# lizhiqi49/threestudio-3dgs

Hardware: AMD Instinct MI355X
Metric: rendered views/sec fwd+bwd @1M Gaussians, 1024², SH=3; 1/2/4/8 GPU (higher is better)
Workload: dtype fp32

## Files before the change

### threestudio-3dgs_amd/csrc/gsr_api.hip

```cpp
#include <stdio.h>
#include <string.h>

#include <cmath>
#include <mutex>
#include <vector>

#include "../../include/gsr.h"
#include "gsr_kernels.h"

using namespace gsr;

static thread_local char g_err[512] = "";

static int fail(int code, const char* fmt, const char* what) {
  snprintf(g_err, sizeof(g_err), fmt, what);
  return code;
}

#define GSR_HIP_CHECK(expr)                                                        \
  do {                                                                             \
    hipError_t e_ = (expr);                                                        \
    if (e_ != hipSuccess) return fail(GSR_EHIP, "HIP error: %s", hipGetErrorString(e_)); \
  } while (0)

// ... 1008 lines not shown
      state->image == nullptr || gr.work == nullptr || dL_dcolor == nullptr || gr.dL_dmeans2D == nullptr ||
      gr.dL_dcolors == nullptr || gr.dL_dopacity == nullptr || gr.dL_dmeans3D == nullptr ||
      state->radii == nullptr || sc.means3D == nullptr)
    return fail(GSR_EINVAL, "%s", "null pointer argument");
  if (sc.shs != nullptr && gr.dL_dsh == nullptr) return fail(GSR_EINVAL, "%s", "dL_dsh required with SHs");
  if (sc.cov3D_precomp == nullptr && (sc.scales == nullptr || sc.rotations == nullptr || gr.dL_dscales == nullptr ||
                                      gr.dL_drotations == nullptr))
    return fail(GSR_EINVAL, "%s", "scales/rotations and their gradients required");
  SetCams cams;
  if (set_cams(sc, cams) != GSR_OK) return GSR_EINVAL;
  SegInfo inst;
  long long total = 0;
  if (inst_segments(V, K, inst, &total) != GSR_OK) return GSR_EINVAL;
  hipStream_t s = (hipStream_t)stream;
  GeomState g = GeomState::carve(state->geom, V, P, nullptr);
  const TilePack tp = set_tile_pack(P, width, height);
  BinningState b = BinningState::carve(state->binning, V, total, inst.blk[V], !tp.packed, nullptr);
  ImageState img = ImageState::carve(state->image, V, width, height, nullptr, true);
  const int gx = div_up(width, GSR_TILE_X), gy = div_up(height, GSR_TILE_Y);
  const size_t HW = (size_t)width * height;
  const int tres = tile_sort_result(width, height);
  const uint32_t* sorted = tp.packed ? b.key[tres] : b.val[tres];
  GaussBackwardArgs a = shared_args(sc, gr);
  if (gr.accumulate != 0 && sc.cov3D_precomp == nullptr && dL_dcov3D == nullptr)
    return fail(GSR_EINVAL, "%s", "accumulate needs dL_dcov3D: it carries the running dL/dcov3D between calls");
  void* work = gr.work;
  if (gr.work_bytes < carry_bytes(P)) return fail(GSR_EINVAL, "%s", "backward work buffer too small");
  const size_t avail = (gr.work_bytes - carry_bytes(P)) & ~(size_t)255;
  float* carry = dL_dcov3D ? dL_dcov3D : (float*)((char*)work + avail);
  bool first = gr.accumulate == 0;
  for (int g0 = 0; g0 < V;) {
    int g1 = g0;
    long long rows = 0;
    while (g1 < V && (g1 == g0 || BackwardState::bytes_for(rows + K[g1], g1 + 1 - g0, P, two) <= avail))
      rows += K[g1++];
    if (BackwardState::bytes_for(rows, g1 - g0, P, two) > avail)
      return fail(GSR_EINVAL, "%s", "backward work buffer smaller than one view's gradient rows");
    BackwardState bw = BackwardState::carve(work, rows, P, two);
    RenderSet rs;
    rs.cbg = comp_bg ? comp_bg + (size_t)g0 * HW * 3 : nullptr;
    rs.comp = nullptr;
    rs.ccolor = color ? color + (size_t)g0 * 3 * HW : nullptr;
    rs.dcbg = dL_dbg ? dL_dbg + (size_t)g0 * HW * 3 : nullptr;
    rs.col2 = two ? gr.colors2 : colors_override;
    rs.col2_rec = g.drange + 130;
    rs.out_col2 = nullptr;
    rs.dpix2 = two ? gr.dL_dcolor2 + (size_t)g0 * 3 * HW : nullptr;
    rs.order = img.order;
    rs.ckpt = !two && colors_override == nullptr && split_fits(V, (size_t)gx * gy) ? img.ckpt : nullptr;
    rs.split_mode = img.split_mode;
    rs.split_items = img.split_items;
    rs.split_cap = img.split_cap;
    rs.split_extra = split_extra(V, (size_t)gx * gy);
    rs.qkeys = tp.qmask ? b.key[tres] : nullptr;
    rs.qbytes = reinterpret_cast<uint8_t*>(b.key[tres ^ 1]);
    rs.V = g1 - g0;
    rs.ochunk = order_chunk(rs.V, gx, gy, false);
    rs.v0 = g0;
    rs.P = P;
    rs.W = width;
    rs.H = height;
    rs.gx = gx;
    rs.gy = gy;
    rs.gmask = tp.gmask;
    ViewGradArgs va;
    va.V = g1 - g0;
    va.v0 = g0;
    va.W = width;
    va.H = height;
    va.gx = gx;
    va.tiles = gx * gy;
    va.cut_in_lds = 0;
    va.items = 0;
    va.g = g;
    va.img = img;
    va.reach = bw.reach;
    va.grow = bw.grow;
    va.dmeans2D = gr.dL_dmeans2D;
    va.vrec = bw.vrec;
    AccumArgs ab;
    ab.V = g1 - g0;
    ab.v0 = g0;
    ab.accumulate = first ? 0 : 1;
    ab.pad_ = 0;
    ab.reach = bw.reach;
    ab.vrec = bw.vrec;
    ab.dcov_carry = carry;
    ab.dcolors2 = two ? gr.dL_dcolors2 : nullptr;
    for (int v = g0; v < g1; ++v) {
      if (bgs[v] == nullptr) return fail(GSR_EINVAL, "%s", "null background");
      rs.inst_start[v - g0] = inst.start[v];
      rs.row_start[v - g0] = inst.start[v] - inst.start[g0];
      rs.bg[v - g0] = bgs[v];
      va.row_start[v - g0] = rs.row_start[v - g0];
      va.cam[v - g0] = cams.c[v];
      ab.campos[v - g0] = cams.c[v].campos;
    }
    {
      PhaseScope ps(GSR_PHASE_RENDER_BWD, s);
      GSR_HIP_CHECK(hipMemsetAsync(bw.reach, 0, sizeof(unsigned long long) * (size_t)P, s));
      launch_render_backward(rs, g, sorted, img, dL_dcolor + (size_t)g0 * 3 * HW,
                             dL_ddepth ? dL_ddepth + (size_t)g0 * HW : nullptr,
                             dL_dalpha ? dL_dalpha + (size_t)g0 * HW : nullptr, bw, s);
    }
    {
      PhaseScope ps(GSR_PHASE_GAUSS_BWD, s);
      const bool last = g1 == V;
      if (last && gr.n_chunks > 0) {
        const int cs = grad_chunk_size(P, gr.n_chunks);
        for (int c = 0; c < gr.n_chunks; ++c) {
          GaussBackwardArgs ac = a;
          ac.g0 = c * cs < P ? c * cs : P;
          ac.g1 = (c + 1) * cs < P ? (c + 1) * cs : P;
          launch_gauss_backward(ac, va, ab, s);
          if (gr.chunk_events[c] != nullptr) GSR_HIP_CHECK(hipEventRecord((hipEvent_t)gr.chunk_events[c], s));
        }
      } else {
        launch_gauss_backward(a, va, ab, s);
      }
    }
    first = false;
    g0 = g1;
  }
  return last_launch();
}

int gsr_grad_chunk_range(int P, int n_chunks, int chunk, int* g0, int* g1) {
  if (P < 0 || n_chunks < 1 || n_chunks > GSR_GRAD_CHUNKS_MAX || chunk < 0 || chunk >= n_chunks || g0 == nullptr ||
      g1 == nullptr)
    return fail(GSR_EINVAL, "%s", "bad gradient chunk query");
  const int cs = grad_chunk_size(P, n_chunks);
  *g0 = chunk * cs < P ? chunk * cs : P;
  *g1 = (chunk + 1) * cs < P ? (chunk + 1) * cs : P;
  return GSR_OK;
}


size_t gsr_geom_bytes(int P) { return gsr_set_geom_bytes(1, P); }
size_t gsr_binning_bytes(int K, int width, int height) {
  SegInfo seg;
  long long total = 0;
  if (K < 0 || inst_segments(1, &K, seg, &total) != GSR_OK) return 0;
  size_t b = 0;
  BinningState::carve(nullptr, 1, total, seg.blk[1], true, &b);
  return b;
}
size_t gsr_image_bytes(int width, int height) { return gsr_set_image_bytes(1, 0, nullptr, width, height, 0); }
size_t gsr_backward_bytes(int P, int K) { return gsr_set_backward_bytes(1, P, &K, 0); }

int gsr_forward_preprocess(int P, int degree, int M, const float* means3D, const float* scales,
                           float scale_modifier, const float* rotations, const float* opacities,
                           const float* shs, const float* colors_precomp, const float* cov3D_precomp,
                           const float* viewmatrix, const float* projmatrix, const float* campos,
                           int width, int height, float tanfovx, float tanfovy, int prefiltered,
                           int* radii, void* geom, void* stream) {
  const gsr_set_scene sc{1, P, degree, M, width, height, prefiltered, scale_modifier, means3D, scales, rotations,
                         opacities, shs, colors_precomp, cov3D_precomp, &viewmatrix, &projmatrix, &campos, nullptr,
                         &tanfovx, &tanfovy};
  const gsr_set_state st{radii, geom, nullptr, nullptr, nullptr};
  return gsr_set_preprocess(&sc, &st, nullptr, stream);
}

int gsr_num_rendered(const void* geom, int P, int* num_rendered, int* num_visible, void* stream) {
  return gsr_set_num_rendered(1, geom, P, num_rendered, num_visible, nullptr, stream);
}

int gsr_forward_render(int P, int K, int width, int height, const float* bg, void* geom,
// ... 81 lines not shown
```

### threestudio-3dgs_amd/csrc/gsr_backward.hip

```cpp
#include <cstdlib>
#include <cstring>

#include "gsr_kernels.h"
#include "gsr_math.h"
#include "gsr_wave.h"

namespace gsr {

struct RowSums {
  float dmx, dmy, dca, dcb, dcc, dop, dcr, dcg, dcbl, ddep;
  float dmx1, dmy1, dr2, dg2, db2;
};

template <bool TWO>
__device__ __forceinline__ RowSums gather_rows(uint32_t idx, const GaussRec& gr, uint32_t i0, int grid_x,
                                               const uint2* cut, const float4* grow) {
  RowSums r = {0.f, 0.f, 0.f, 0.f, 0.f, 0.f, 0.f, 0.f, 0.f, 0.f, 0.f, 0.f, 0.f, 0.f, 0.f};
  constexpr int RW = TWO ? 4 : 3;
  const uint4 gd = gr.d;
  const float4 ga = gr.a, gb = gr.b;
  const uint32_t dkey = __float_as_uint(gb.z);
  const int xmin = gd.x & 0xffff, ymin = gd.x >> 16, xmax = gd.y & 0xffff, ymax = gd.y >> 16;
  const int w = xmax - xmin;
  const SpanPrep sp = span_prep(ga.x, ga.y, ga.z, ga.w, gb.x, gb.y);
// ... 253 lines not shown
#pragma unroll
  for (int it = 0; it < GSR_VG_ITEMS; ++it) {
    const int local = it * 256 + t;
    const int idx = slice + local;
    const bool valid = it < items && idx < a.g1;
    const bool rch = valid && (va.reach[idx] & vbit) != 0ull;
    if (valid && !rch) {
      float* m2 = va.dmeans2D + 3 * ((size_t)vg * a.P + idx);
      m2[0] = 0.f;
      m2[1] = 0.f;
      m2[2] = 0.f;
    }
    const unsigned long long bal = __ballot(rch);
    if (rch) list[cnt + mask_rank(bal)] = (uint16_t)local;
    cnt += __popcll(bal);
  }
  asm volatile("s_waitcnt lgkmcnt(0)" ::: "memory");
  GaussRec nrec;
  uint32_t ngo = 0u;
  int nidx = 0;
  if (lane < cnt) {
    nidx = slice + list[lane];
    const size_t o0 = (size_t)vg * a.P + nidx;
    nrec = va.g.rec[o0], ngo = va.g.goff[o0];
  }
#pragma unroll 1
  for (int i = lane; i - lane < cnt; i += 64) {
    if (i >= cnt) break;
    const int idx = nidx;
    const size_t o = (size_t)vg * a.P + idx;
    const GaussRec gr = nrec;
    const uint32_t go = ngo;
    if (i + 64 < cnt) {
      nidx = slice + list[i + 64];
      const size_t on = (size_t)vg * a.P + nidx;
      nrec = va.g.rec[on], ngo = va.g.goff[on];
    }
    float* m2 = va.dmeans2D + 3 * o;
    float4* rec = recv + (size_t)idx * (RS / 4);
    const uint32_t clamp_bits = gr.d.w;
    const RowSums r = gather_rows<TWO>((uint32_t)idx, gr, go, va.gx, cut, grow);
    bool reached = (r.dmx != 0.f) | (r.dmy != 0.f) | (r.dca != 0.f) | (r.dcb != 0.f) | (r.dcc != 0.f) |
                   (r.dop != 0.f) | (r.dcr != 0.f) | (r.dcg != 0.f) | (r.dcbl != 0.f) | (r.ddep != 0.f);
    if (TWO) reached = reached | (r.dr2 != 0.f) | (r.dg2 != 0.f) | (r.db2 != 0.f);
    if (!reached) {
      m2[0] = 0.f;
      m2[1] = 0.f;
      m2[2] = 0.f;
#pragma unroll
      for (int q = 0; q < RS / 4; ++q)
        rec[q] = q == 3 ? make_float4(0.f, __uint_as_float(clamp_bits), 0.f, 0.f) : make_float4(0.f, 0.f, 0.f, 0.f);
      continue;
    }
    m2[0] = TWO ? r.dmx1 : r.dmx;
    m2[1] = TWO ? r.dmy1 : r.dmy;
    m2[2] = 0.f;
    const float3 mean = make_float3(a.means3D[3 * idx], a.means3D[3 * idx + 1], a.means3D[3 * idx + 2]);
    float cov3D[6];
    if (a.cov3D_precomp) {
#pragma unroll
      for (int k = 0; k < 6; ++k) cov3D[k] = a.cov3D_precomp[6 * idx + k];
    } else {
      const float3 scale = make_float3(a.scales[3 * idx], a.scales[3 * idx + 1], a.scales[3 * idx + 2]);
      const float4 rot = make_float4(a.rotations[4 * idx], a.rotations[4 * idx + 1], a.rotations[4 * idx + 2],
                                     a.rotations[4 * idx + 3]);
      cov3d_from_scale_rot(scale, a.scale_modifier, rot, cov3D);
    }
    float dcv[6];
    float3 dm;
    cov2d_backward(mean, cov3D, vgm, r.dca, r.dcb, r.dcc, dcv, dm);
    proj_backward(mean, projm, r.dmx, r.dmy, dm);
    dm.x += viewm[2] * r.ddep;
    dm.y += viewm[6] * r.ddep;
    dm.z += viewm[10] * r.ddep;
    const float f[GSR_REC_STRIDE2] = {dm.x,   dm.y,  dm.z,  dcv[0], dcv[1], dcv[2], dcv[3],
                                      dcv[4], dcv[5], r.dcr, r.dcg,  r.dcbl, r.dop,  __uint_as_float(clamp_bits),
                                      r.dr2,  r.dg2, r.db2, 0.f,   0.f,    0.f};
#pragma unroll
    for (int q = 0; q < RS / 4; ++q) rec[q] = make_float4(f[4 * q], f[4 * q + 1], f[4 * q + 2], f[4 * q + 3]);
  }
}

__attribute__((amdgpu_waves_per_eu(3, 8)))
__global__ __launch_bounds__(256) void k_gauss_accum(GaussBackwardArgs a, AccumArgs b) {
  extern __shared__ __attribute__((aligned(16))) float s_sh[];
  const int t = threadIdx.x;
  const int block0 = a.g0 + blockIdx.x * 256;
  const int idx = block0 + t;
  const int nblk = min(256, a.g1 - block0);
  const int F = 3 * a.M;
  const int S = sh_lds_stride(a.M);
  const bool has_sh = a.shs != nullptr && F > 0;
  const bool acc = b.accumulate != 0;
  const float invF = has_sh ? 1.0f / (float)F : 0.0f;
  __shared__ uint8_t s_rl[256];
  __shared__ int s_wcnt[4];
  const unsigned long long reach_word = idx < a.g1 ? b.reach[idx] : 0ull;
  const bool reached = reach_word != 0ull;
  int nr = 0;
  if (has_sh) {
    const unsigned long long bal = __ballot(reached);
    const int w = t >> 6;
    if ((t & 63) == 0) s_wcnt[w] = (int)__popcll(bal);
    __syncthreads();
    int base = 0;
    for (int k = 0; k < 4; ++k) {
      base += k < w ? s_wcnt[k] : 0;
      nr += s_wcnt[k];
    }
    if (reached) s_rl[base + mask_rank(bal)] = (uint8_t)t;
    __syncthreads();
    const int cnt = nr * F;
    for (int e = t; e < cnt; e += 256) {
      const int r = (int)(((float)e + 0.5f) * invF);
      const int tl = s_rl[r];
      const int k = e - r * F;
      s_sh[tl * S + k] = a.shs[(size_t)(block0 + tl) * F + k];
    }
    __syncthreads();
  }
  if (idx < a.g1 && !reached) {
    if (!acc) {
      for (int k = 0; k < 3; ++k) a.dL_dmeans3D[3 * idx + k] = 0.f;
      a.dL_dopacity[idx] = 0.f;
      if (a.dL_dcolors)
        for (int k = 0; k < 3; ++k) a.dL_dcolors[3 * idx + k] = 0.f;
      if (b.dcolors2)
        for (int k = 0; k < 3; ++k) b.dcolors2[3 * idx + k] = 0.f;
      if (b.dcov_carry)
        for (int k = 0; k < 6; ++k) b.dcov_carry[6 * idx + k] = 0.f;
      if (a.dL_dcov3D && a.dL_dcov3D != b.dcov_carry)
        for (int k = 0; k < 6; ++k) a.dL_dcov3D[6 * idx + k] = 0.f;
      if (!a.cov3D_precomp && a.dL_dscales) {
        for (int k = 0; k < 3; ++k) a.dL_dscales[3 * idx + k] = 0.f;
        for (int k = 0; k < 4; ++k) a.dL_drotations[4 * idx + k] = 0.f;
      }
      if (has_sh) {
        float* row = s_sh + t * S;
        for (int k = 0; k < F; ++k) row[k] = 0.f;
      }
    }
  } else if (idx < a.g1) {
    const float3 mean = make_float3(a.means3D[3 * idx], a.means3D[3 * idx + 1], a.means3D[3 * idx + 2]);
    float3 dmean = make_float3(0.f, 0.f, 0.f);
    float dcov[6] = {0.f, 0.f, 0.f, 0.f, 0.f, 0.f};
    float dop = 0.f, dcr = 0.f, dcg = 0.f, dcb = 0.f;
    float dsh[48];
#pragma unroll
    for (int k = 0; k < 48; ++k) dsh[k] = 0.f;
    if (acc) {
      dmean = make_float3(a.dL_dmeans3D[3 * idx], a.dL_dmeans3D[3 * idx + 1], a.dL_dmeans3D[3 * idx + 2]);
      dop = a.dL_dopacity[idx];
      if (a.dL_dcolors) dcr = a.dL_dcolors[3 * idx], dcg = a.dL_dcolors[3 * idx + 1], dcb = a.dL_dcolors[3 * idx + 2];
      if (b.dcov_carry)
#pragma unroll
        for (int k = 0; k < 6; ++k) dcov[k] = b.dcov_carry[6 * idx + k];
      if (has_sh) {
        const float* prev = a.dL_dsh + (size_t)idx * F;
#pragma unroll
        for (int k = 0; k < 48; ++k)
          if (k < F) dsh[k] = prev[k];
      }
    }
    const float* sh_row = has_sh ? s_sh + t * S : nullptr;
    const int RS = b.dcolors2 ? GSR_REC_STRIDE2 : GSR_REC_STRIDE;
    float d2[3] = {0.f, 0.f, 0.f};
    if (b.dcolors2 && acc)
      for (int k = 0; k < 3; ++k) d2[k] = b.dcolors2[3 * idx + k];
    unsigned long long pending = reach_word;
    auto next_view = [&]() -> int {
      if (pending == 0ull) return -1;
      const int v = __builtin_ctzll(pending);
      pending &= pending - 1ull;
      return v;
    };
    auto load = [&](float4 (&f)[4], int vl) {
      const float4* src = reinterpret_cast<const float4*>(b.vrec + ((size_t)vl * a.P + idx) * RS);
#pragma unroll
      for (int q = 0; q < 4; ++q) f[q] = src[q];
    };
    auto process = [&](const float4 (&f4)[4], int vl) {
      const float f[16] = {f4[0].x, f4[0].y, f4[0].z, f4[0].w, f4[1].x, f4[1].y, f4[1].z, f4[1].w,
                           f4[2].x, f4[2].y, f4[2].z, f4[2].w, f4[3].x, f4[3].y, f4[3].z, f4[3].w};
      dmean.x += f[0];
      dmean.y += f[1];
      dmean.z += f[2];
#pragma unroll
      for (int k = 0; k < 6; ++k) dcov[k] += f[3 + k];
      dcr += f[9];
      dcg += f[10];
      dcb += f[11];
      dop += f[12];
      if (b.dcolors2) {
        d2[0] += f[14];
        d2[1] += f[15];
        d2[2] += b.vrec[((size_t)vl * a.P + idx) * RS + 16];
      }
      if (has_sh && ((f[9] != 0.f) | (f[10] != 0.f) | (f[11] != 0.f))) {
        const uint32_t cl = __float_as_uint(f[13]);
        const float3 dRGB = make_float3((cl & 1u) ? 0.f : f[9], (cl & 2u) ? 0.f : f[10], (cl & 4u) ? 0.f : f[11]);
        const float* shv = sh_row;
        typedef __attribute__((address_space(4))) const float* cfptr;
        const float cpos[3] = {((cfptr)b.campos[vl])[0], ((cfptr)b.campos[vl])[1], ((cfptr)b.campos[vl])[2]};
        sh_backward(a.deg, a.M, shv, dsh, dRGB, mean, cpos, dmean);
      }
    };
    float4 fa[4], fb[4];
    int va_ = next_view(), vb_ = next_view();
    if (va_ >= 0) load(fa, va_);
    if (vb_ >= 0) load(fb, vb_);
    for (;;) {
      if (va_ < 0) break;
      process(fa, va_);
      va_ = next_view();
      if (va_ >= 0) load(fa, va_);
      if (vb_ < 0) break;
      process(fb, vb_);
      vb_ = next_view();
      if (vb_ >= 0) load(fb, vb_);
    }
    a.dL_dmeans3D[3 * idx] = dmean.x;
    a.dL_dmeans3D[3 * idx + 1] = dmean.y;
    a.dL_dmeans3D[3 * idx + 2] = dmean.z;
    a.dL_dopacity[idx] = dop;
    if (a.dL_dcolors) {
      a.dL_dcolors[3 * idx] = dcr;
      a.dL_dcolors[3 * idx + 1] = dcg;
      a.dL_dcolors[3 * idx + 2] = dcb;
    }
    if (b.dcolors2)
      for (int k = 0; k < 3; ++k) b.dcolors2[3 * idx + k] = d2[k];
    if (b.dcov_carry)
      for (int k = 0; k < 6; ++k) b.dcov_carry[6 * idx + k] = dcov[k];
    if (a.dL_dcov3D && a.dL_dcov3D != b.dcov_carry)
      for (int k = 0; k < 6; ++k) a.dL_dcov3D[6 * idx + k] = dcov[k];
    if (!a.cov3D_precomp && a.dL_dscales) {
      const float3 scale = make_float3(a.scales[3 * idx], a.scales[3 * idx + 1], a.scales[3 * idx + 2]);
      const float4 rot = make_float4(a.rotations[4 * idx], a.rotations[4 * idx + 1], a.rotations[4 * idx + 2],
                                     a.rotations[4 * idx + 3]);
      float ds[3], dq[4];
      scale_rot_backward(scale, rot, a.scale_modifier, dcov, ds, dq);
      for (int k = 0; k < 3; ++k) a.dL_dscales[3 * idx + k] = ds[k];
      for (int k = 0; k < 4; ++k) a.dL_drotations[4 * idx + k] = dq[k];
    }
    if (has_sh) {
      float* row = s_sh + t * S;
      float4* row4w = reinterpret_cast<float4*>(row);
#pragma unroll
      for (int c = 0; c < 12; ++c)
        if (4 * c < F) row4w[c] = make_float4(dsh[4 * c], dsh[4 * c + 1], dsh[4 * c + 2], dsh[4 * c + 3]);
      for (int k = 48; k < F; ++k) row[k] = 0.f;
    }
  }
  if (has_sh) {
    __syncthreads();
    if (!acc) {
      float* dst = a.dL_dsh + (size_t)block0 * F;
      const int cnt = nblk * F;
      for (int e = t; e < cnt; e += 256) {
        const int te = (int)(((float)e + 0.5f) * invF);
        dst[e] = s_sh[te * S + (e - te * F)];
      }
    } else {
      const int cnt = nr * F;
      for (int e = t; e < cnt; e += 256) {
        const int r = (int)(((float)e + 0.5f) * invF);
        const int tl = s_rl[r];
        const int k = e - r * F;
        a.dL_dsh[(size_t)(block0 + tl) * F + k] = s_sh[tl * S + k];
      }
    }
  }
}

template <bool TWO>
__global__ __launch_bounds__(256) void k_gauss_fused(GaussBackwardArgs a, ViewGradArgs va, AccumArgs b) {
  const int idx = a.g0 + blockIdx.x * 256 + threadIdx.x;
  const bool valid = idx < a.g1;
  const int ix = valid ? idx : a.g0;
  const bool acc = b.accumulate != 0;
  const unsigned long long reach_word = valid ? va.reach[ix] : 0ull;
  float3 dmean = make_float3(0.f, 0.f, 0.f);
  float dcov[6] = {0.f, 0.f, 0.f, 0.f, 0.f, 0.f};
  float dop = 0.f, dcr = 0.f, dcg = 0.f, dcb = 0.f;
  float d2[3] = {0.f, 0.f, 0.f};
  if (valid && acc) {
    dmean = make_float3(a.dL_dmeans3D[3 * idx], a.dL_dmeans3D[3 * idx + 1], a.dL_dmeans3D[3 * idx + 2]);
    dop = a.dL_dopacity[idx];
    if (a.dL_dcolors) dcr = a.dL_dcolors[3 * idx], dcg = a.dL_dcolors[3 * idx + 1], dcb = a.dL_dcolors[3 * idx + 2];
    if (b.dcov_carry)
#pragma unroll
      for (int k = 0; k < 6; ++k) dcov[k] = b.dcov_carry[6 * idx + k];
    if (TWO)
      for (int k = 0; k < 3; ++k) d2[k] = b.dcolors2[3 * idx + k];
  }
  const float3 mean = make_float3(a.means3D[3 * ix], a.means3D[3 * ix + 1], a.means3D[3 * ix + 2]);
  float cov3D[6];
  if (reach_word != 0ull) {
    if (a.cov3D_precomp) {
#pragma unroll
      for (int k = 0; k < 6; ++k) cov3D[k] = a.cov3D_precomp[6 * ix + k];
    } else {
      const float3 scale = make_float3(a.scales[3 * ix], a.scales[3 * ix + 1], a.scales[3 * ix + 2]);
      const float4 rot = make_float4(a.rotations[4 * ix], a.rotations[4 * ix + 1], a.rotations[4 * ix + 2],
                                     a.rotations[4 * ix + 3]);
      cov3d_from_scale_rot(scale, a.scale_modifier, rot, cov3D);
    }
  }
  GaussRec nrec;
  uint32_t ngo = 0u;
  auto fetch = [&](int vl) {
    const size_t o = (size_t)(va.v0 + vl) * a.P + ix;
    nrec = va.g.rec[o];
    ngo = va.g.goff[o];
  };
  const int vfirst = reach_word != 0ull ? (int)__builtin_ctzll(reach_word) : va.V;
  if (vfirst < va.V) fetch(vfirst);
#pragma unroll 1
  for (int vl = 0; vl < va.V; ++vl) {
    const int vg = va.v0 + vl;
    float* m2 = va.dmeans2D + 3 * ((size_t)vg * a.P + ix);
    if (!((reach_word >> vl) & 1ull)) {
      if (valid) m2[0] = 0.f, m2[1] = 0.f, m2[2] = 0.f;
      continue;
    }
    const GaussRec gr = nrec;
    const uint32_t go = ngo;
    const unsigned long long later = reach_word & ~((2ull << vl) - 1ull);
    if (later != 0ull) fetch((int)__builtin_ctzll(later));
    const ViewCam& cam = va.cam[vl];
    typedef __attribute__((address_space(4))) const float* cfptr;
    float viewm[16], projm[16];
#pragma unroll
    for (int i = 0; i < 16; ++i) viewm[i] = ((cfptr)cam.view)[i], projm[i] = ((cfptr)cam.proj)[i];
    ViewGeom vgm;
    vgm.view = viewm;
    vgm.proj = projm;
    vgm.tanx = cam.tanx;
    vgm.tany = cam.tany;
    vgm.fy = va.H / (2.0f * cam.tany);
    vgm.fx = va.W / (2.0f * cam.tanx);
    const float4* grow = va.grow + (size_t)(TWO ? 4 : 3) * va.row_start[vl];
    const uint2* cut = va.img.cut + (size_t)vg * va.tiles;
    const RowSums r = gather_rows<TWO>((uint32_t)ix, gr, go, va.gx, cut, grow);
    bool reached = (r.dmx != 0.f) | (r.dmy != 0.f) | (r.dca != 0.f) | (r.dcb != 0.f) | (r.dcc != 0.f) |
                   (r.dop != 0.f) | (r.dcr != 0.f) | (r.dcg != 0.f) | (r.dcbl != 0.f) | (r.ddep != 0.f);
    if (TWO) reached = reached | (r.dr2 != 0.f) | (r.dg2 != 0.f) | (r.db2 != 0.f);
    if (!reached) {
      if (valid) m2[0] = 0.f, m2[1] = 0.f, m2[2] = 0.f;
      continue;
    }
    if (valid) {
      m2[0] = TWO ? r.dmx1 : r.dmx;
      m2[1] = TWO ? r.dmy1 : r.dmy;
      m2[2] = 0.f;
    }
    float dcv[6];
    float3 dm;
    cov2d_backward(mean, cov3D, vgm, r.dca, r.dcb, r.dcc, dcv, dm);
    proj_backward(mean, projm, r.dmx, r.dmy, dm);
    dm.x += viewm[2] * r.ddep;
    dm.y += viewm[6] * r.ddep;
    dm.z += viewm[10] * r.ddep;
    dmean.x += dm.x;
    dmean.y += dm.y;
    dmean.z += dm.z;
#pragma unroll
    for (int k = 0; k < 6; ++k) dcov[k] += dcv[k];
    dcr += r.dcr;
    dcg += r.dcg;
    dcb += r.dcbl;
    dop += r.dop;
    if (TWO) {
      d2[0] += r.dr2;
      d2[1] += r.dg2;
      d2[2] += r.db2;
    }
  }
  if (!valid) return;
  a.dL_dmeans3D[3 * idx] = dmean.x;
  a.dL_dmeans3D[3 * idx + 1] = dmean.y;
  a.dL_dmeans3D[3 * idx + 2] = dmean.z;
  a.dL_dopacity[idx] = dop;
  if (a.dL_dcolors) {
    a.dL_dcolors[3 * idx] = dcr;
    a.dL_dcolors[3 * idx + 1] = dcg;
    a.dL_dcolors[3 * idx + 2] = dcb;
  }
  if (TWO)
    for (int k = 0; k < 3; ++k) b.dcolors2[3 * idx + k] = d2[k];
  if (b.dcov_carry)
    for (int k = 0; k < 6; ++k) b.dcov_carry[6 * idx + k] = dcov[k];
  if (a.dL_dcov3D && a.dL_dcov3D != b.dcov_carry)
    for (int k = 0; k < 6; ++k) a.dL_dcov3D[6 * idx + k] = dcov[k];
  if (!a.cov3D_precomp && a.dL_dscales) {
    const float3 scale = make_float3(a.scales[3 * idx], a.scales[3 * idx + 1], a.scales[3 * idx + 2]);
    const float4 rot = make_float4(a.rotations[4 * idx], a.rotations[4 * idx + 1], a.rotations[4 * idx + 2],
                                   a.rotations[4 * idx + 3]);
    float ds[3], dq[4];
    scale_rot_backward(scale, rot, a.scale_modifier, dcov, ds, dq);
    for (int k = 0; k < 3; ++k) a.dL_dscales[3 * idx + k] = ds[k];
    for (int k = 0; k < 4; ++k) a.dL_drotations[4 * idx + k] = dq[k];
  }
}

static bool gauss_fused_on(const GaussBackwardArgs& a) {
  if (a.shs != nullptr && a.M > 0) return false;
  const char* e = getenv("GSR_GAUSS_FUSED");
  return !(e != nullptr && strcmp(e, "0") == 0);
}

#define GSR_CUT_LDS_MAX (48 * 1024)

void launch_gauss_backward(const GaussBackwardArgs& a, ViewGradArgs va, const AccumArgs& b, hipStream_t stream) {
  const int n = a.g1 - a.g0;
  if (n <= 0 || va.V <= 0) return;
  if (gauss_fused_on(a)) {
    auto kern = b.dcolors2 ? k_gauss_fused<true> : k_gauss_fused<false>;
    hipLaunchKernelGGL(kern, dim3(div_up(n, 256)), dim3(256), 0, stream, a, va, b);
    return;
  }
  const size_t cut_bytes = sizeof(uint2) * (size_t)va.tiles;
  va.cut_in_lds = cut_bytes <= GSR_CUT_LDS_MAX ? 1 : 0;
  va.items = GSR_VG_ITEMS;
  while (va.items > 2 && (long long)va.V * div_up(n, 256 * va.items) < 1024) va.items >>= 1;
  const dim3 vg_grid(va.V * div_up(n, 256 * va.items));
  auto vg_kern = b.dcolors2 ? (va.cut_in_lds ? k_view_grad<true, true> : k_view_grad<true, false>)
                            : (va.cut_in_lds ? k_view_grad<false, true> : k_view_grad<false, false>);
  hipLaunchKernelGGL(vg_kern, vg_grid, dim3(256), va.cut_in_lds ? cut_bytes : 0, stream, a, va);
  const size_t lds = (a.shs && a.M > 0) ? (size_t)256 * sh_lds_stride(a.M) * sizeof(float) : 0;
  hipLaunchKernelGGL(k_gauss_accum, dim3(div_up(n, 256)), dim3(256), lds, stream, a, b);
}

}
```

### threestudio-3dgs_amd/csrc/gsr_kernels.h

```cpp
#pragma once

#include "gsr_common.h"

namespace gsr {

int seg_sort(uint32_t* keys[2], uint32_t* vals[2], bool vals_identity, SegInfo seg, int bit_lo, int key_bits,
             uint32_t* counts, uint32_t* totals, hipStream_t stream, int max_bits = GSR_RADIX_BITS);
int sort_rank_mode();

struct PreprocessArgs {
  int V, P, deg, M;
  const float *means3D, *scales, *rotations, *opacities, *shs, *colors_precomp, *cov3D_precomp;
  float scale_modifier;
  int W, H;
  int* radii;
  const float* col2;
};
void launch_preprocess(const PreprocessArgs& a, const SetCams& cams, const GeomState& g, hipStream_t stream);

void launch_binning_counts(int V, int P, const GeomState& g, hipStream_t stream);
void launch_emit(int V, int P, int W, const GeomState& g, const SegInfo& inst, const TilePack& tp, uint32_t* keys,
                 uint32_t* vals, hipStream_t stream);
void launch_tile_ranges(SegInfo inst, int n_tiles, const TilePack& tp, const uint32_t* keys, uint2* ranges,
                        hipStream_t stream);
void launch_mark_visible(int P, const float* means3D, const float* view, const float* proj,
                         uint8_t* present, hipStream_t stream);

__device__ __forceinline__ float quad_form(float a, float b, float c, float u, float v) {
  return fmaf(a * u, u, fmaf(2.0f * b * u, v, c * v * v));
}
__device__ __forceinline__ bool quadrant_hit(const float4 r0, const float4 r1, float qx, float qy) {
  const float o = r1.y;
  if (!(o >= GSR_ALPHA_MIN * 0.9999f)) return false;
  const float a = r0.z, b = r0.w, c = r1.x;
  if (!(a > 0.0f && c > 0.0f && a * c - b * b > 0.0f)) return true;
  const float tau = fmaxf(0.0f, __logf(255.0f * o));
  const float thr = 2.0f * (tau * 1.002f + 2e-3f);
  const float u1 = r0.x - qx, u0 = u1 - 7.0f;
  const float v1 = r0.y - qy, v0 = v1 - 7.0f;
  if (u0 <= 0.0f && u1 >= 0.0f && v0 <= 0.0f && v1 >= 0.0f) return true;
  const float ia = 1.0f / a, ic = 1.0f / c;
  const float q0 = quad_form(a, b, c, u0, fminf(fmaxf(-b * u0 * ic, v0), v1));
  const float q1 = quad_form(a, b, c, u1, fminf(fmaxf(-b * u1 * ic, v0), v1));
  const float q2 = quad_form(a, b, c, fminf(fmaxf(-b * v0 * ia, u0), u1), v0);
  const float q3 = quad_form(a, b, c, fminf(fmaxf(-b * v1 * ia, u0), u1), v1);
  const float qmin = fminf(fminf(q0, q1), fminf(q2, q3));
  return qmin * 0.998f <= thr;
}

struct RenderSet {
  int V, v0, P, W, H, gx, gy;
  uint32_t gmask;
  uint32_t inst_start[GSR_SET_MAX];
  uint32_t row_start[GSR_SET_MAX];
  const float* bg[GSR_SET_MAX];
  const float* cbg;
  float* comp;
  const float* ccolor;
  float* dcbg;
  const float* col2;
  float* out_col2;
  const float* dpix2;
  const uint32_t* order;
  int ochunk;
  float* ckpt;
  const uint32_t* split_mode;
  const uint32_t* col2_rec;
  uint32_t* split_items;
  uint32_t* split_cap;
  int split_extra;
  const uint32_t* qkeys;
  uint8_t* qbytes;
};
bool split_on(int V, int P, int width, int height, long long instances);
bool fwd_tile_chosen(long long instances, long long gaussians, int views);
int order_chunk(int V, int gx, int gy, bool forward);
const char* blend_kernel_name(int which);
inline bool split_forward(int V, int P, int width, int height, long long instances, bool two_colors) {
  return !two_colors && split_on(V, P, width, height, instances);
}
void launch_tile_order(int V, int gx, int gy, const uint2* ranges, uint32_t* order, hipStream_t stream);
void launch_render_forward(const RenderSet& rs, const GeomState& g, const uint32_t* sorted_gauss,
                           const ImageState& img, float* out_color, float* out_depth, float* out_alpha,
                           long long instances, hipStream_t stream);
void launch_render_backward(const RenderSet& rs, const GeomState& g, const uint32_t* sorted_gauss,
                            const ImageState& img, const float* dL_dcolor, const float* dL_ddepth,
                            const float* dL_dalpha, const BackwardState& bw, hipStream_t stream);

struct GaussBackwardArgs {
  int P, deg, M;
  int g0, g1;
  const float *means3D, *scales, *rotations, *shs, *cov3D_precomp;
  float scale_modifier;
  float *dL_dcolors, *dL_dopacity, *dL_dmeans3D, *dL_dcov3D, *dL_dsh, *dL_dscales, *dL_drotations;
};
struct ViewGradArgs {
  int V, v0, W, H, gx, tiles, cut_in_lds, items;
  GeomState g;
  ImageState img;
  const unsigned long long* reach;
  const float4* grow;
  float* dmeans2D;
  float* vrec;
  uint32_t row_start[GSR_SET_MAX];
  ViewCam cam[GSR_SET_MAX];
};
struct AccumArgs {
  int V, v0, accumulate, pad_;
  const unsigned long long* reach;
  const float* vrec;
  float* dcov_carry;
  float* dcolors2;
  const float* campos[GSR_SET_MAX];
};
void launch_composite_fwd(int V, size_t HW, const float* color, const float* alpha, const float* bg, int layout,
                          float* out, hipStream_t stream);
void launch_composite_bwd(int V, size_t HW, const float* dout, const float* color, const float* alpha,
                          const float* bg, int layout, float* dcolor, float* dalpha, float* dbg,
                          hipStream_t stream);
void launch_normal_map_fwd(int V, size_t HW, const float* normal, const float* alpha, float* out, hipStream_t stream);
void launch_normal_map_bwd(int V, size_t HW, const float* dout, const float* normal, const float* alpha,
                           float* dnormal, float* dalpha, hipStream_t stream);
struct ShadeArgs {
  int V, v0, H, W, flags, bg_layout;
  const float* color;
  const float* depth;
  const float* alpha;
  const float* rays_o;
  const float* rays_d;
  const float* bg;
  const float* light;
  const float* pred_normal;
  float ka[GSR_SET_MAX][3], kd[GSR_SET_MAX][3];
  int mode[GSR_SET_MAX];
  float* render;
  float* nmap;
  float* unit;
  float* depth_out;
};
struct ShadeGrads {
  const float* d_render;
  const float* d_nmap;
  const float* d_unit;
  const float* d_depth_out;
  float* d_color;
  float* d_depth;
  float* d_alpha;
  float* d_bg;
};
void launch_shade_fwd(const ShadeArgs& A, hipStream_t stream);
void launch_shade_bwd(const ShadeArgs& A, const ShadeGrads& G, hipStream_t stream);
size_t knn_workspace_bytes(int P);
int launch_knn_mean_dist(int P, const float* points, float* out, void* workspace, hipStream_t stream);
int launch_knn_points(int P, int K, const float* points, float* dists, long long* idx, void* workspace,
                      hipStream_t stream);
struct FieldCall {
  int M, K, N, R;
  const float* x;
  const long long *nbr, *row;
  const float *centers, *inv_sr, *strengths, *min_scale;
  float density_factor;
};
size_t field_workspace_bytes(long long M, int K, int N);
int field_gauss_lanes(long long M, int K, int N);
void launch_field_forward(const FieldCall& c, float* density, float* beta_avg, float* op, void* workspace,
                          hipStream_t stream);
int launch_field_backward(const FieldCall& c, const float* g_density, const float* g_beta, const float* g_op, float* dx,
                          float* dcenters, float* dinv_sr, float* dstrengths, float* dmin_scale, void* workspace,
                          hipStream_t stream);
struct NormalCall {
  int M, K, N, R;
  const float* x;
  const long long *own, *nbr;
  int per_sample;
  const float *centers, *normals, *min_scale, *op;
};
size_t normal_workspace_bytes(long long M, int K, int N);
int normal_gauss_lanes(long long M, int K, int N);
void launch_normal_forward(const NormalCall& c, float* loss, float* rec, void* workspace, hipStream_t stream);
int launch_normal_backward(const NormalCall& c, const float* rec, const float* g_loss, float* dnormals,
                           void* workspace, hipStream_t stream);
struct MeshCall {
  int V, F, G;
  const float* verts;
  const int* faces;
  const float *cplx, *log_scales;
};
size_t mesh_workspace_bytes(int F, int V);
void launch_mesh_forward(const MeshCall& c, const float* bary, float thickness, float* xyz, float* scaling,
                         float* rotation, float* normals, hipStream_t stream);
void launch_mesh_backward(const MeshCall& c, const float* bary, const int* corner_order, const int* vert_offsets,
// ... 38 lines not shown
```

Measured before the change: 3988.

## Balance per-Gaussian accumulation work across wavefronts by sorting on reached-view count

The Gaussian gradient accumulation kernel drops from 256-thread blocks to single-wave 64-thread blocks. Four of these waves share each 256-Gaussian chunk, and each wave recomputes a counting sort of the chunk by popcount of the per-Gaussian view-reach mask. Gaussians that touch a similar number of views therefore land in the same wave, which is meant to cut time lanes spend idle behind the longest per-view loop. SH staging in LDS is compacted to reached Gaussians only, and unreached SH gradients are zeroed directly in global memory. The cost is the sort done redundantly in each block, scattered rather than contiguous SH writes, and smaller blocks. A diagnostic script measuring lane imbalance is also added.

```diff
diff --git a/profiles/diag_lane_balance.py b/profiles/diag_lane_balance.py
--- /dev/null
+++ b/profiles/diag_lane_balance.py
@@ -0,0 +1,130 @@
+import ctypes
+import json
+import os
+import sys
+
+ROOT = os.path.dirname(os.path.dirname(os.path.abspath(__file__)))
+sys.path.insert(0, os.path.join(ROOT, "threestudio-3dgs_amd"))
+sys.path.insert(0, ROOT)
+
+import numpy as np
+import torch
+
+import bench
+import gsr_synthetic as gs
+from diff_gaussian_rasterization import _C
+
+
+def popcount64(x: torch.Tensor) -> torch.Tensor:
+    m1, m2, m4 = 0x5555555555555555, 0x3333333333333333, 0x0F0F0F0F0F0F0F0F
+    lo = x & 0xFFFFFFFF
+    hi = (x >> 32) & 0xFFFFFFFF
+    out = 0
+    for h in (lo, hi):
+        h = h - ((h >> 1) & (m1 & 0xFFFFFFFF))
+        h = (h & (m2 & 0xFFFFFFFF)) + ((h >> 2) & (m2 & 0xFFFFFFFF))
+        h = (h + (h >> 4)) & (m4 & 0xFFFFFFFF)
+        out = out + ((h * 0x01010101) >> 24 & 0xFF)
+    return out
+
+
+def pad_to(x: torch.Tensor, m: int) -> torch.Tensor:
+    n = (-x.shape[-1]) % m
+    return torch.nn.functional.pad(x, (0, n)) if n else x
+
+
+def main():
+    lib = _C.load_library()
+    dev = torch.device("cuda", 0)
+    V, R, P = 64, 1024, 1_000_000
+    scene = gs.make_scene(P, sh_degree=3, seed=0)
+    rep = bench.Replica(scene, dev)
+    cams = bench.build_views(V, R, dev)
+    bg0 = torch.zeros(3, device=dev)
+    settings = [bench.settings_for(rep, c, bg0) for c in cams]
+    gen = torch.Generator(device=dev).manual_seed(7)
+    bg_img = torch.rand((V, R, R, 3), generator=gen, device=dev)
+    ups = [torch.randn((V, 3, R, R), generator=gen, device=dev), torch.randn((V, 1, R, R), generator=gen, device=dev),
+           torch.randn((V, 1, R, R), generator=gen, device=dev)]
+
+    hip = ctypes.CDLL("libamdhip64.so")
+    hip.hipMemcpy.argtypes = [ctypes.c_void_p, ctypes.c_void_p, ctypes.c_size_t, ctypes.c_int]
+    inner = lib.gsr_set_backward
+    seen = []
+
+    def set_backward(sc, st, g, stream):
+        rc = inner(sc, st, g, stream)
+        if rc == 0:
+            reach = np.zeros(sc.P, np.int64)
+            assert hip.hipMemcpy(reach.ctypes.data, g.work, 8 * sc.P, 2) == 0
+            rows, vis = geom_state(lib, st.geom, sc.V, sc.P, dev)
+            seen.append((reach, rows, vis, sc.V))
+        return rc
+
+    lib.gsr_set_backward = set_backward
+    c, d, a, _ = bench.render_views(rep, settings, bg_img)
+    torch.autograd.backward((c, d, a), ups)
+    torch.cuda.synchronize()
+    lib.gsr_set_backward = inner
+    assert len(seen) == 1, f"expected one set, saw {len(seen)} backward calls"
+    reach, rows, vis, Vs = seen[0]
+
+    pc = popcount64(torch.from_numpy(reach).to(dev))
+    group_views = (int(np.bitwise_or.reduce(reach)) & (2 ** 64 - 1)).bit_length()
+    hist = torch.bincount(pc, minlength=65).cpu().tolist()
+    waves = pad_to(pc, 64).view(-1, 64)
+    wave_max = int(waves.max(1).values.sum())
+    blocks = pad_to(pc, 256).view(-1, 256)
+    ordered = blocks.sort(1, descending=True).values.reshape(-1, 64)
+    wave_max_ordered = int(ordered.max(1).values.sum())
+    n_waves = waves.shape[0]
+    total = int(pc.sum())
+
+    r = pad_to(torch.where(vis, rows, torch.zeros_like(rows)), 64).view(Vs, -1, 64)
+    row_sum = int(r.sum())
+    row_max64 = int(r.max(2).values.sum()) * 64
+    items = int(vis.sum())
+
+    out = {
+        "workload": f"bench.py default: 1M Gaussians, {R}x{R}, SH3, {V}-view set, fused background composite",
+        "build_id": _C.build_id(lib),
+        "views": Vs,
+        "gauss_accum": {
+            "views_in_last_group": group_views,
+            "popcount_histogram": hist,
+            "mean_popcount": total / P,
+            "reached_fraction": float((pc > 0).float().mean()),
+            "waves": n_waves,
+            "sum_wave_max": wave_max,
+            "sum_wave_max_ordered_256": wave_max_ordered,
+            "sum_wave_mean": total / 64.0,
+            "max_over_ordered": wave_max / max(1, wave_max_ordered),
+            "max_over_mean": wave_max / max(1.0, total / 64.0),
+        },
+        "preprocess": {
+            "visible_nonzero_area": items,
+            "mean_rows": row_sum / max(1, items),
+            "sum_rows": row_sum,
+            "sum_wave_max_x64": row_max64,
+            "max64_over_sum": row_max64 / max(1, row_sum),
+            "mean_wave_max": row_max64 / 64 / (Vs * r.shape[1]),
+            "mean_wave_rounds_of_64": float(((r.sum(2) + 63) // 64).float().mean()),
+        },
+    }
+    path = sys.argv[1] if len(sys.argv) > 1 else os.path.join(ROOT, "profiles", "lane_balance.json")
+    with open(path, "w") as f:
+        json.dump(out, f, indent=1)
+    print(json.dumps(out, indent=1))
+
+
+def geom_state(lib, geom, V, P, dev):
+    rec = torch.zeros((V, P, 16), dtype=torch.float32, device=dev)
+    tiles = torch.zeros((V, P, 2), dtype=torch.int32, device=dev)
+    _C._check(lib.gsr_set_gauss_state(V, geom, P, _C._ptr(rec), _C._ptr(tiles), _C._stream(dev)))
+    d = rec.view(torch.int32)
+    rows = ((d[:, :, 13] >> 16) & 0xFFFF) - ((d[:, :, 12] >> 16) & 0xFFFF)
+    return rows.long(), tiles[:, :, 0] > 0
+
+
+if __name__ == "__main__":
+    main()
diff --git a/threestudio-3dgs_amd/csrc/gsr_api.hip b/threestudio-3dgs_amd/csrc/gsr_api.hip
--- a/threestudio-3dgs_amd/csrc/gsr_api.hip
+++ b/threestudio-3dgs_amd/csrc/gsr_api.hip
@@ -1114,7 +1114,7 @@
     ab.V = g1 - g0;
     ab.v0 = g0;
     ab.accumulate = first ? 0 : 1;
-    ab.pad_ = 0;
+    ab.balance = 0;
     ab.reach = bw.reach;
     ab.vrec = bw.vrec;
     ab.dcov_carry = carry;
diff --git a/threestudio-3dgs_amd/csrc/gsr_backward.hip b/threestudio-3dgs_amd/csrc/gsr_backward.hip
--- a/threestudio-3dgs_amd/csrc/gsr_backward.hip
+++ b/threestudio-3dgs_amd/csrc/gsr_backward.hip
@@ -359,44 +359,83 @@
 }
 
 __attribute__((amdgpu_waves_per_eu(3, 8)))
-__global__ __launch_bounds__(256) void k_gauss_accum(GaussBackwardArgs a, AccumArgs b) {
+__global__ __launch_bounds__(64) void k_gauss_accum(GaussBackwardArgs a, AccumArgs b) {
   extern __shared__ __attribute__((aligned(16))) float s_sh[];
-  const int t = threadIdx.x;
-  const int block0 = a.g0 + blockIdx.x * 256;
-  const int idx = block0 + t;
-  const int nblk = min(256, a.g1 - block0);
+  const int lane = threadIdx.x;
+  const int block0 = a.g0 + (int)(blockIdx.x >> 2) * 256;
+  const int p = (int)(blockIdx.x & 3u);
   const int F = 3 * a.M;
   const int S = sh_lds_stride(a.M);
   const bool has_sh = a.shs != nullptr && F > 0;
   const bool acc = b.accumulate != 0;
   const float invF = has_sh ? 1.0f / (float)F : 0.0f;
-  __shared__ uint8_t s_rl[256];
-  __shared__ int s_wcnt[4];
-  const unsigned long long reach_word = idx < a.g1 ? b.reach[idx] : 0ull;
+  __shared__ uint8_t s_perm[256];
+  __shared__ uint8_t s_rl[64];
+  __shared__ uint8_t s_zl[64];
+  if (b.balance) {
+    __shared__ uint16_t s_cnt[4][66];
+    __shared__ uint16_t s_base[66];
+    for (int k = lane; k < 4 * 66; k += 64) (&s_cnt[0][0])[k] = 0;
+    __syncthreads();
+    uint32_t key[4], below[4];
+#pragma unroll
+    for (int j = 0; j < 4; ++j) {
+      const int i = block0 + 64 * j + lane;
+      const unsigned long long word = i < a.g1 ? b.reach[i] : 0ull;
+      key[j] = 64u - (uint32_t)__popcll(word);
+      const unsigned long long peers = match_digit(key[j], 7, true);
+      below[j] = mask_rank(peers);
+      if (below[j] == 0u) s_cnt[j][key[j]] = (uint16_t)__popcll(peers);
+    }
+    __syncthreads();
+    {
+      const uint32_t tot = (uint32_t)s_cnt[0][lane] + s_cnt[1][lane] + s_cnt[2][lane] + s_cnt[3][lane];
+      const uint32_t incl = wave_incl_sum_dpp(tot);
+      s_base[lane] = (uint16_t)(incl - tot);
+      if (lane == 63) s_base[64] = (uint16_t)incl;
+    }
+    __syncthreads();
+#pragma unroll
+    for (int j = 0; j < 4; ++j) {
+      uint32_t rank = (uint32_t)s_base[key[j]] + below[j];
+      for (int k = 0; k < j; ++k) rank += (uint32_t)s_cnt[k][key[j]];
+      s_perm[rank] = (uint8_t)(64 * j + lane);
+    }
+    __syncthreads();
+  }
+  const int own = b.balance ? (int)s_perm[64 * p + lane] : 64 * p + lane;
+  const int idx = block0 + own;
+  const bool valid = idx < a.g1;
+  if (__ballot(valid) == 0ull) return;
+  const unsigned long long reach_word = valid ? b.reach[idx] : 0ull;
   const bool reached = reach_word != 0ull;
-  int nr = 0;
+  const unsigned long long bal = __ballot(reached);
+  const int np = (int)__popcll(bal);
+  const int slot = (int)mask_rank(bal);
   if (has_sh) {
-    const unsigned long long bal = __ballot(reached);
-    const int w = t >> 6;
-    if ((t & 63) == 0) s_wcnt[w] = (int)__popcll(bal);
+    const unsigned long long zbal = __ballot(valid && !reached);
+    if (reached) s_rl[slot] = (uint8_t)own;
+    if (valid && !reached) s_zl[mask_rank(zbal)] = (uint8_t)own;
     __syncthreads();
-    int base = 0;
-    for (int k = 0; k < 4; ++k) {
-      base += k < w ? s_wcnt[k] : 0;
-      nr += s_wcnt[k];
-    }
-    if (reached) s_rl[base + mask_rank(bal)] = (uint8_t)t;
-    __syncthreads();
-    const int cnt = nr * F;
-    for (int e = t; e < cnt; e += 256) {
+    const int cnt = np * F;
+#pragma unroll 4
+    for (int e = lane; e < cnt; e += 64) {
       const int r = (int)(((float)e + 0.5f) * invF);
       const int tl = s_rl[r];
       const int k = e - r * F;
-      s_sh[tl * S + k] = a.shs[(size_t)(block0 + tl) * F + k];
+      s_sh[r * S + k] = a.shs[(size_t)(block0 + tl) * F + k];
+    }
+    if (!acc) {
+      const int zcnt = (int)__popcll(zbal) * F;
+      for (int e = lane; e < zcnt; e += 64) {
+        const int r = (int)(((float)e + 0.5f) * invF);
+        const int tl = s_zl[r];
+        a.dL_dsh[(size_t)(block0 + tl) * F + (e - r * F)] = 0.f;
+      }
     }
     __syncthreads();
   }
-  if (idx < a.g1 && !reached) {
+  if (valid && !reached) {
     if (!acc) {
       for (int k = 0; k < 3; ++k) a.dL_dmeans3D[3 * idx + k] = 0.f;
       a.dL_dopacity[idx] = 0.f;
@@ -412,12 +451,8 @@
         for (int k = 0; k < 3; ++k) a.dL_dscales[3 * idx + k] = 0.f;
         for (int k = 0; k < 4; ++k) a.dL_drotations[4 * idx + k] = 0.f;
       }
-      if (has_sh) {
-        float* row = s_sh + t * S;
-        for (int k = 0; k < F; ++k) row[k] = 0.f;
-      }
-    }
-  } else if (idx < a.g1) {
+    }
+  } else if (valid) {
     const float3 mean = make_float3(a.means3D[3 * idx], a.means3D[3 * idx + 1], a.means3D[3 * idx + 2]);
     float3 dmean = make_float3(0.f, 0.f, 0.f);
     float dcov[6] = {0.f, 0.f, 0.f, 0.f, 0.f, 0.f};
@@ -439,7 +474,7 @@
           if (k < F) dsh[k] = prev[k];
       }
     }
-    const float* sh_row = has_sh ? s_sh + t * S : nullptr;
+    const float* sh_row = has_sh ? s_sh + slot * S : nullptr;
     const int RS = b.dcolors2 ? GSR_REC_STRIDE2 : GSR_REC_STRIDE;
     float d2[3] = {0.f, 0.f, 0.f};
     if (b.dcolors2 && acc)
@@ -521,7 +556,7 @@
       for (int k = 0; k < 4; ++k) a.dL_drotations[4 * idx + k] = dq[k];
     }
     if (has_sh) {
-      float* row = s_sh + t * S;
+      float* row = s_sh + slot * S;
       float4* row4w = reinterpret_cast<float4*>(row);
 #pragma unroll
       for (int c = 0; c < 12; ++c)
@@ -531,21 +566,12 @@
   }
   if (has_sh) {
     __syncthreads();
-    if (!acc) {
-      float* dst = a.dL_dsh + (size_t)block0 * F;
-      const int cnt = nblk * F;
-      for (int e = t; e < cnt; e += 256) {
-        const int te = (int)(((float)e + 0.5f) * invF);
-        dst[e] = s_sh[te * S + (e - te * F)];
-      }
-    } else {
-      const int cnt = nr * F;
-      for (int e = t; e < cnt; e += 256) {
-        const int r = (int)(((float)e + 0.5f) * invF);
-        const int tl = s_rl[r];
-        const int k = e - r * F;
-        a.dL_dsh[(size_t)(block0 + tl) * F + k] = s_sh[tl * S + k];
-      }
+    const int cnt = np * F;
+    for (int e = lane; e < cnt; e += 64) {
+      const int r = (int)(((float)e + 0.5f) * invF);
+      const int tl = s_rl[r];
+      const int k = e - r * F;
+      a.dL_dsh[(size_t)(block0 + tl) * F + k] = s_sh[r * S + k];
     }
   }
 }
@@ -687,6 +713,14 @@
   return !(e != nullptr && strcmp(e, "0") == 0);
 }
 
+static bool accum_balance_on() {
+  static const bool on = [] {
+    const char* e = getenv("GSR_ACCUM_BALANCE");
+    return !(e != nullptr && strcmp(e, "0") == 0);
+  }();
+  return on;
+}
+
 #define GSR_CUT_LDS_MAX (48 * 1024)
 
 void launch_gauss_backward(const GaussBackwardArgs& a, ViewGradArgs va, const AccumArgs& b, hipStream_t stream) {
@@ -705,8 +739,10 @@
   auto vg_kern = b.dcolors2 ? (va.cut_in_lds ? k_view_grad<true, true> : k_view_grad<true, false>)
                             : (va.cut_in_lds ? k_view_grad<false, true> : k_view_grad<false, false>);
   hipLaunchKernelGGL(vg_kern, vg_grid, dim3(256), va.cut_in_lds ? cut_bytes : 0, stream, a, va);
-  const size_t lds = (a.shs && a.M > 0) ? (size_t)256 * sh_lds_stride(a.M) * sizeof(float) : 0;
-  hipLaunchKernelGGL(k_gauss_accum, dim3(div_up(n, 256)), dim3(256), lds, stream, a, b);
-}
-
-}
+  const size_t lds = (a.shs && a.M > 0) ? (size_t)64 * sh_lds_stride(a.M) * sizeof(float) : 0;
+  AccumArgs bb = b;
+  bb.balance = accum_balance_on() ? 1 : 0;
+  hipLaunchKernelGGL(k_gauss_accum, dim3(4 * div_up(n, 256)), dim3(64), lds, stream, a, bb);
+}
+
+}
diff --git a/threestudio-3dgs_amd/csrc/gsr_kernels.h b/threestudio-3dgs_amd/csrc/gsr_kernels.h
--- a/threestudio-3dgs_amd/csrc/gsr_kernels.h
+++ b/threestudio-3dgs_amd/csrc/gsr_kernels.h
@@ -106,7 +106,8 @@
   ViewCam cam[GSR_SET_MAX];
 };
 struct AccumArgs {
-  int V, v0, accumulate, pad_;
+  int V, v0, accumulate;
+  int balance;
   const unsigned long long* reach;
   const float* vrec;
   float* dcov_carry;
```

After: 3856. 3.3% lower.
